# Komputerowe-Projektowanie-Lekow/pmarlo

Measured on AMD Instinct MI355X. Metric: frames/sec featurize->TICA->k-means->T-matrix, 1Mx64 synth; ITS rel-err, higher is better.
Workload: dtype f64; 1 GPU; synthetic 1000000 frames x 64 f32 features per GPU (AR(1) latents), TICA->10, k=500 (10 Lloyd iterations), lag=10, row-normalised T; frames_per_gpu=1000000, features=64, tica_dim=10, k=500, lag=10, kmeans_iters=10, parallelism=shards1

## Files before the change

### pmarlo_amd/csrc/kmeans.hip

```cpp
#include "common.h"
#include "wave.h"

#include <algorithm>
#include <cstdlib>

namespace {

constexpr int kThreads = 256;

template <typename T>
__device__ __forceinline__ double load_as_f64(const T* p) { return (double)(*p); }

struct FitState {
    double scale;
    double inv_scale;
    double absmax;
    double shift2;
    double tol2;
    double done;
    double n_iter;
    double inertia;
};

__device__ __forceinline__ long long to_fixed(double v, double scale) { return __double2ll_rn(v * scale); }
// ... 673 lines not shown

template <typename T, int KS, bool ACCUM>
msm_status launch_mfma(msm_ctx* ctx, const T* x, int64_t n, int d, int64_t ld, const double* centers, int k,
                       const double* mean, const double* stdv, int32_t* labels, double* mindist, const FitState* st,
                       unsigned long long* sums, unsigned long long* counts) {
    constexpr int NF = KS <= 16 ? 2 : 1;
    constexpr int kMT = KS <= 4 ? kMTNarrow : kMTWide;
    constexpr int TS = KS * 64 + 1;
    const size_t acc_bytes = ACCUM ? (size_t)k * (d + 1) * sizeof(unsigned long long) : 0;
    const int lds_acc = ACCUM && acc_bytes <= 64 * 1024;
    const size_t tile_budget = 150 * 1024 - (lds_acc ? acc_bytes : 0);
    int tile_k = (int)(tile_budget / ((TS + 16) * sizeof(double))) * 16;
    const int k16 = (k + 15) & ~15;
    if (tile_k > k16) tile_k = k16;
    if (tile_k < 16) tile_k = 16;
    if (tile_k < k16 && tile_k >= 32) tile_k &= ~31;
    const size_t lds = (size_t)(tile_k / 16) * (TS + 16) * sizeof(double) + (lds_acc ? acc_bytes : 0);
    const int64_t n_units = (n + 16 * NF - 1) / (16 * NF);
    const int waves = kMT / 64;
    const int grid = (int)std::min<int64_t>((n_units + waves - 1) / waves, (int64_t)ctx->n_cu);
    const bool multi = k > tile_k;
    const bool foldm = (d & 3) != 0;
    auto kern = multi ? (foldm ? kmeans_mfma_kernel<T, KS, NF, kMT, ACCUM, true, true>
                               : kmeans_mfma_kernel<T, KS, NF, kMT, ACCUM, false, true>)
                      : (foldm ? kmeans_mfma_kernel<T, KS, NF, kMT, ACCUM, true, false>
                               : kmeans_mfma_kernel<T, KS, NF, kMT, ACCUM, false, false>);
    double* chalf_g = nullptr;
    double* tile_img = nullptr;
    if (multi) {
        const size_t n_tiles_all = (size_t)k16 / 16;
        const size_t img_doubles = (n_tiles_all * TS + 1) & ~(size_t)1;
        msm_status rs = msm_reserve_aux(ctx, (img_doubles + k16) * sizeof(double));
        if (rs != MSM_OK) return rs;
        tile_img = (double*)ctx->aux;
        chalf_g = tile_img + img_doubles;
        if (foldm)
            hipLaunchKernelGGL((pack_tiles_kernel<KS, true>), dim3((unsigned)n_tiles_all), dim3(64), 0, ctx->stream, centers,
                               k, d, tile_img, chalf_g);
        else
            hipLaunchKernelGGL((pack_tiles_kernel<KS, false>), dim3((unsigned)n_tiles_all), dim3(64), 0, ctx->stream, centers,
                               k, d, tile_img, chalf_g);
    } else if (KS > 8) {
        msm_status rs = msm_reserve_aux(ctx, (size_t)k * sizeof(double));
        if (rs != MSM_OK) return rs;
        chalf_g = (double*)ctx->aux;
        hipLaunchKernelGGL(chalf_kernel, dim3((k + 255) / 256), dim3(256), 0, ctx->stream, centers, k, d, chalf_g);
    }
    if (getenv("MSM_KMEANS_DEBUG"))
        fprintf(stderr, "msm_kmeans: fp64 T=%s n=%lld d=%d k=%d KS=%d NF=%d MT=%d ACCUM=%d FOLD=%d MULTI=%d tile_k=%d lds_acc=%d grid=%d lds=%zu\n",
                sizeof(T) == 4 ? "f32" : "f64", (long long)n, d, k, KS, NF, kMT, (int)ACCUM, (int)foldm, (int)multi, tile_k,
                lds_acc, grid, lds);
    if (lds > 48 * 1024)
        MSM_HIP(ctx, hipFuncSetAttribute((const void*)kern, hipFuncAttributeMaxDynamicSharedMemorySize, (int)lds));
    hipLaunchKernelGGL(kern, dim3(grid), dim3(kMT), lds, ctx->stream, x, n, d, ld, centers, k, mean, stdv, tile_k,
                       labels, mindist, st, sums, counts, lds_acc, (const double*)chalf_g, (const double*)tile_img);
    MSM_CHECK_LAUNCH(ctx);
    return MSM_OK;
}

__global__ void mfma_bf16_probe_kernel(const uint16_t* __restrict__ A, const uint16_t* __restrict__ B,
                                       const float* __restrict__ C, float* __restrict__ D) {
    const int l = threadIdx.x, i = l & 15, q = l >> 4;
    A += (size_t)blockIdx.x * 512;
    B += (size_t)blockIdx.x * 512;
    C += (size_t)blockIdx.x * 256;
    D += (size_t)blockIdx.x * 256;
    v8bf a, b;
    for (int j = 0; j < 8; ++j) {
        a[j] = __builtin_bit_cast(__bf16, A[i * 32 + 8 * q + j]);
        b[j] = __builtin_bit_cast(__bf16, B[(8 * q + j) * 16 + i]);
    }
    v4f32 c;
    for (int r = 0; r < 4; ++r) c[r] = C[(4 * q + r) * 16 + i];
    c = __builtin_amdgcn_mfma_f32_16x16x32_bf16(a, b, c, 0, 0, 0);
    for (int r = 0; r < 4; ++r) D[(4 * q + r) * 16 + i] = c[r];
}

__global__ void mfma_f16_probe_kernel(const uint16_t* __restrict__ A, const uint16_t* __restrict__ B,
                                      const float* __restrict__ C, float* __restrict__ D) {
    const int l = threadIdx.x, i = l & 15, q = l >> 4;
    A += (size_t)blockIdx.x * 512;
    B += (size_t)blockIdx.x * 512;
    C += (size_t)blockIdx.x * 256;
    D += (size_t)blockIdx.x * 256;
    v8h a, b;
    for (int j = 0; j < 8; ++j) {
        a[j] = __builtin_bit_cast(_Float16, A[i * 32 + 8 * q + j]);
        b[j] = __builtin_bit_cast(_Float16, B[(8 * q + j) * 16 + i]);
    }
    v4f32 c;
    for (int r = 0; r < 4; ++r) c[r] = C[(4 * q + r) * 16 + i];
    c = __builtin_amdgcn_mfma_f32_16x16x32_f16(a, b, c, 0, 0, 0);
    for (int r = 0; r < 4; ++r) D[(4 * q + r) * 16 + i] = c[r];
}

bool filter_enabled() {
    static const bool on = [] {
        const char* e = getenv("MSM_KMEANS_FILTER");
        return !(e && e[0] == '0');
    }();
    return on;
}

size_t filter_image_bytes(int64_t n, int) { return (size_t)((n + 63) & ~(int64_t)63) * 16 * kFilterRowQ + 16; }

template <typename T>
msm_status launch_pack(msm_ctx* ctx, const T* x, int64_t n, int d, int64_t ld, const double* mean, const double* stdv,
                       const double* absmax, uint4* image) {
    const unsigned grid = (unsigned)((n + 255) / 256);
    if (!absmax) {
        uint4* tail = image + (size_t)((n + 63) & ~(int64_t)63) * kFilterRowQ;
        MSM_HIP(ctx, hipMemsetAsync(tail, 0, 8, ctx->stream));
        const int g = (int)std::min<int64_t>((n * d + 256 * 8 - 1) / (256 * 8), (int64_t)ctx->n_cu * 8);
        hipLaunchKernelGGL(filter_absmax_kernel<T>, dim3(g), dim3(256), 0, ctx->stream, x, n, d, ld, mean, stdv,
                           (unsigned long long*)tail);
        MSM_CHECK_LAUNCH(ctx);
        absmax = (const double*)tail;
    }
    const int dense = ld == d && ((uintptr_t)x & 15) == 0;
#define MSM_PACK_CASE(D)                                                                                              \
    case D:                                                                                                           \
        hipLaunchKernelGGL((kmeans_pack_kernel<T, D>), dim3(grid), dim3(256), 0, ctx->stream, x, n, ld, mean, stdv, absmax, \
                           image, dense);                                                                             \
        break
    switch (d) {
        MSM_PACK_CASE(1); MSM_PACK_CASE(2); MSM_PACK_CASE(3); MSM_PACK_CASE(4); MSM_PACK_CASE(5);
        MSM_PACK_CASE(6); MSM_PACK_CASE(7); MSM_PACK_CASE(8); MSM_PACK_CASE(9); MSM_PACK_CASE(10);
        default: return msm_fail(ctx, MSM_ERR_UNSUPPORTED, "k-means frame images need d <= %d (got %d)", kFilterMaxD, d);
    }
#undef MSM_PACK_CASE
    MSM_CHECK_LAUNCH(ctx);
    return MSM_OK;
}

msm_status filter_stats_buffer(msm_ctx* ctx, unsigned long long** out) {
    static_assert(sizeof(unsigned long long) == 8, "");
    if (!ctx->km_stats) {
        if (ctx->capturing) { *out = nullptr; return MSM_OK; }
        MSM_HIP(ctx, hipMalloc(&ctx->km_stats, 16));
        MSM_HIP(ctx, hipMemsetAsync(ctx->km_stats, 0, 16, ctx->stream));
    }
    *out = (unsigned long long*)ctx->km_stats;
    return MSM_OK;
}

template <typename T, int DP, bool ACCUM>
msm_status launch_filter_dp(msm_ctx* ctx, const T* x, int64_t n, int d, int64_t ld, const double* centers, int k,
                            const double* mean, const double* stdv, const uint4* image, int32_t* labels, double* mindist,
                            const FitState* st, unsigned long long* sums, unsigned long long* counts, double* upd_centers) {
    constexpr int NF = 4;
    const size_t lds = filter_lds_bytes(k, d, ACCUM);
    msm_status rs;
    const int64_t n_units = (n + 16 * NF - 1) / (16 * NF);
    const int kWaves = filter_waves(DP, ACCUM);
    const int grid = (int)std::min<int64_t>((n_units + kWaves - 1) / kWaves, (int64_t)ctx->n_cu);
    unsigned long long* stats = nullptr;
    rs = filter_stats_buffer(ctx, &stats);
    if (rs != MSM_OK) return rs;
    auto kern = mean ? kmeans_filter_kernel<T, DP, NF, ACCUM, true> : kmeans_filter_kernel<T, DP, NF, ACCUM, false>;
    if (lds > 48 * 1024)
        MSM_HIP(ctx, hipFuncSetAttribute((const void*)kern, hipFuncAttributeMaxDynamicSharedMemorySize, (int)lds));
    hipLaunchKernelGGL(kern, dim3(grid), dim3(64 * kWaves), lds, ctx->stream, x, n, d, ld, k, mean, stdv, image, centers,
                       labels, mindist, st, sums, counts, stats, stats ? upd_centers : nullptr,
                       stats ? (unsigned int*)(stats + 1) : nullptr);
    MSM_CHECK_LAUNCH(ctx);
    return MSM_OK;
}

template <typename T, bool ACCUM>
msm_status launch_filter(msm_ctx* ctx, const T* x, int64_t n, int d, int64_t ld, const double* centers, int k,
                         const double* mean, const double* stdv, const uint4* image, int32_t* labels, double* mindist,
                         const FitState* st, unsigned long long* sums, unsigned long long* counts, double* upd_centers) {
    if (filter_dp(d) == 4)
        return launch_filter_dp<T, 4, ACCUM>(ctx, x, n, d, ld, centers, k, mean, stdv, image, labels, mindist, st, sums,
                                             counts, upd_centers);
    return launch_filter_dp<T, 10, ACCUM>(ctx, x, n, d, ld, centers, k, mean, stdv, image, labels, mindist, st, sums, counts,
                                          upd_centers);
}

bool filter_fits(int k, int d, bool accum) { return filter_enabled() && d <= kFilterMaxD && filter_lds_bytes(k, d, accum) != 0; }

template <typename T, bool ACCUM>
msm_status dispatch_mfma(msm_ctx* ctx, const T* x, int64_t n, int d, int64_t ld, const double* centers, int k,
                         const double* mean, const double* stdv, int32_t* labels, double* mindist, const FitState* st,
                         unsigned long long* sums, unsigned long long* counts, const void* image = nullptr,
                         double* upd_centers = nullptr, bool* folded = nullptr) {
    if (folded) *folded = false;
    if (filter_fits(k, d, ACCUM)) {
        if (getenv("MSM_KMEANS_DEBUG"))
            fprintf(stderr, "msm_kmeans: filter T=%s n=%lld d=%d k=%d ACCUM=%d\n", sizeof(T) == 4 ? "f32" : "f64", (long long)n,
                    d, k, (int)ACCUM);
        if (!image) {
            msm_status rs = msm_reserve_km_image(ctx, filter_image_bytes(n, d));
            if (rs != MSM_OK) return rs;
            rs = launch_pack<T>(ctx, x, n, d, ld, mean, stdv, nullptr, (uint4*)ctx->km_image);
            if (rs != MSM_OK) return rs;
            image = ctx->km_image;
        }
        if (upd_centers && !(ACCUM && (int64_t)k * d <= kUpdateWide && (ctx->km_stats || !ctx->capturing))) upd_centers = nullptr;
        if (folded) *folded = upd_centers != nullptr;
        return launch_filter<T, ACCUM>(ctx, x, n, d, ld, centers, k, mean, stdv, (const uint4*)image, labels, mindist, st,
                                       sums, counts, upd_centers);
    }
#define MSM_MFMA_CASE(KSV) \
    if (d <= 4 * KSV)      \
        return launch_mfma<T, KSV, ACCUM>(ctx, x, n, d, ld, centers, k, mean, stdv, labels, mindist, st, sums, counts)
    MSM_MFMA_CASE(1);
    MSM_MFMA_CASE(2);
    MSM_MFMA_CASE(3);
    MSM_MFMA_CASE(4);
    MSM_MFMA_CASE(6);
    MSM_MFMA_CASE(8);
    MSM_MFMA_CASE(12);
    MSM_MFMA_CASE(16);
    MSM_MFMA_CASE(24);
    MSM_MFMA_CASE(32);
    MSM_MFMA_CASE(48);
    MSM_MFMA_CASE(64);
#undef MSM_MFMA_CASE
    return msm_fail(ctx, MSM_ERR_UNSUPPORTED, "k-means: d=%d > 256 not supported", d);
}

msm_status mfma_probe(msm_ctx* ctx, bool f16, const uint16_t* h_a, const uint16_t* h_b, const float* h_c, float* h_d,
                      int n_tiles) {
    if (!ctx) return MSM_ERR_INVALID;
    MSM_REQUIRE(ctx, n_tiles >= 1 && h_a && h_b && h_c && h_d, "msm_mfma_probe: bad arguments");
    const size_t na = (size_t)n_tiles * 512 * sizeof(uint16_t), nc = (size_t)n_tiles * 256 * sizeof(float);
    msm_status rs = msm_reserve_scratch(ctx, 2 * na + 2 * nc);
    if (rs != MSM_OK) return rs;
    unsigned char* base = (unsigned char*)ctx->scratch;
    uint16_t* d_a = (uint16_t*)base;
    uint16_t* d_b = (uint16_t*)(base + na);
    float* d_c = (float*)(base + 2 * na);
    float* d_d = (float*)(base + 2 * na + nc);
    MSM_HIP(ctx, hipMemcpyAsync(d_a, h_a, na, hipMemcpyHostToDevice, ctx->stream));
    MSM_HIP(ctx, hipMemcpyAsync(d_b, h_b, na, hipMemcpyHostToDevice, ctx->stream));
    MSM_HIP(ctx, hipMemcpyAsync(d_c, h_c, nc, hipMemcpyHostToDevice, ctx->stream));
    if (f16)
        hipLaunchKernelGGL(mfma_f16_probe_kernel, dim3((unsigned)n_tiles), dim3(64), 0, ctx->stream, d_a, d_b, d_c, d_d);
    else
        hipLaunchKernelGGL(mfma_bf16_probe_kernel, dim3((unsigned)n_tiles), dim3(64), 0, ctx->stream, d_a, d_b, d_c, d_d);
    MSM_CHECK_LAUNCH(ctx);
    MSM_HIP(ctx, hipMemcpyAsync(h_d, d_d, nc, hipMemcpyDeviceToHost, ctx->stream));
    MSM_HIP(ctx, hipStreamSynchronize(ctx->stream));
    return MSM_OK;
}

}

extern "C" {

static msm_status kmeans_assign_impl(msm_ctx* ctx, const void* d_x, msm_dtype dtype, int64_t n, int d, int64_t ld,
                                     const double* d_centers, int k, const double* d_mean, const double* d_std,
                                     const void* d_image, int32_t* d_labels, double* d_mindist) {
    if (!ctx) return MSM_ERR_INVALID;
    MSM_REQUIRE(ctx, n >= 0 && d >= 1 && k >= 1, "msm_kmeans_assign: need n >= 0, d >= 1, k >= 1");
    MSM_REQUIRE(ctx, ld >= d, "msm_kmeans_assign: ld (%lld) < d (%d)", (long long)ld, d);
    MSM_REQUIRE(ctx, (d_mean == nullptr) == (d_std == nullptr),
                "msm_kmeans_assign: mean and std must both be given or both be NULL");
    MSM_REQUIRE(ctx, dtype == MSM_F32 || dtype == MSM_F64, "msm_kmeans_assign: bad dtype");
    if (n == 0) return MSM_OK;
    MSM_REQUIRE(ctx, d_x && d_centers && d_labels, "msm_kmeans_assign: NULL pointer");
    if (dtype == MSM_F32)
        return dispatch_mfma<float, false>(ctx, (const float*)d_x, n, d, ld, d_centers, k, d_mean, d_std, d_labels,
                                           d_mindist, nullptr, nullptr, nullptr, d_image);
    return dispatch_mfma<double, false>(ctx, (const double*)d_x, n, d, ld, d_centers, k, d_mean, d_std, d_labels,
                                        d_mindist, nullptr, nullptr, nullptr, d_image);
}

msm_status msm_kmeans_assign(msm_ctx* ctx, const void* d_x, msm_dtype dtype, int64_t n, int d, int64_t ld,
                             const double* d_centers, int k, const double* d_mean, const double* d_std,
                             int32_t* d_labels, double* d_mindist) {
    return kmeans_assign_impl(ctx, d_x, dtype, n, d, ld, d_centers, k, d_mean, d_std, nullptr, d_labels, d_mindist);
}

msm_status msm_kmeans_assign_packed(msm_ctx* ctx, const void* d_x, msm_dtype dtype, int64_t n, int d, int64_t ld,
                                    const double* d_centers, int k, const double* d_mean, const double* d_std,
                                    const void* d_image, int32_t* d_labels, double* d_mindist) {
    return kmeans_assign_impl(ctx, d_x, dtype, n, d, ld, d_centers, k, d_mean, d_std, d_image, d_labels, d_mindist);
}

msm_status msm_kmeans_image_bytes(int64_t n, int d, size_t* out_bytes) {
    if (!out_bytes || n < 0 || d < 1) return MSM_ERR_INVALID;
    *out_bytes = d <= kFilterMaxD ? filter_image_bytes(n, d) : 0;
    return MSM_OK;
}

msm_status msm_kmeans_pack(msm_ctx* ctx, const void* d_x, msm_dtype dtype, int64_t n, int d, int64_t ld,
                           const double* d_mean, const double* d_std, void* d_image) {
    return msm_kmeans_pack_bounded(ctx, d_x, dtype, n, d, ld, d_mean, d_std, nullptr, d_image);
}

msm_status msm_kmeans_pack_bounded(msm_ctx* ctx, const void* d_x, msm_dtype dtype, int64_t n, int d, int64_t ld,
                                   const double* d_mean, const double* d_std, const double* d_absmax, void* d_image) {
    if (!ctx) return MSM_ERR_INVALID;
    MSM_REQUIRE(ctx, n >= 0 && d >= 1 && d <= kFilterMaxD && ld >= d, "msm_kmeans_pack: need 1 <= d <= %d, ld >= d",
                kFilterMaxD);
    MSM_REQUIRE(ctx, (d_mean == nullptr) == (d_std == nullptr), "msm_kmeans_pack: mean/std must come together");
    MSM_REQUIRE(ctx, dtype == MSM_F32 || dtype == MSM_F64, "msm_kmeans_pack: bad dtype");
    if (n == 0) return MSM_OK;
    MSM_REQUIRE(ctx, d_x && d_image, "msm_kmeans_pack: NULL pointer");
    MSM_REQUIRE(ctx, ((uintptr_t)d_image & 15) == 0, "msm_kmeans_pack: the image must be 16-byte aligned");
    if (dtype == MSM_F32)
        return launch_pack<float>(ctx, (const float*)d_x, n, d, ld, d_mean, d_std, d_absmax, (uint4*)d_image);
    return launch_pack<double>(ctx, (const double*)d_x, n, d, ld, d_mean, d_std, d_absmax, (uint4*)d_image);
}

// ... 191 lines not shown
```

### pmarlo_amd/csrc/kmeans_filter.h

```cpp
#pragma once

typedef __bf16 v8bf __attribute__((ext_vector_type(8)));
typedef _Float16 v8h __attribute__((ext_vector_type(8)));
typedef float v4f32 __attribute__((ext_vector_type(4)));

#ifdef MSM_KMF_WAVES
__host__ __device__ constexpr int filter_waves(int, bool) { return MSM_KMF_WAVES; }
#else
__host__ __device__ constexpr int filter_waves(int dp, bool heavy) { return dp == 10 && heavy ? 12 : 16; }
#endif
constexpr int kFilterMaxD = 10;
constexpr int kFilterRowQ = 3;
constexpr double kFilterHi = 1e18;
constexpr double kFilterScaledHi = 16384.0;
constexpr double kF16MinNormal = 6.103515625e-05;
constexpr int kFilterScaleTop = 13;
constexpr double kFilterKappa = 52.0 * 5.9604644775390625e-08;
constexpr float kPickEps = 20.0f * 5.9604644775390625e-08f;
constexpr float kPickFloor = 1e-30f;
constexpr float kUp20 = 1.0f + 9.5367431640625e-07f;
constexpr double kUp20d = 1.0 + 9.5367431640625e-07;

__host__ __device__ inline int filter_scale_exp(double amax) {
    if (!(amax > 0.0) || !(amax <= 1.7976931348623157e308)) return 0;
    const int q = ilogb(amax) + 1;
    const int e = kFilterScaleTop - q;
    return e < -60 ? -60 : (e > 60 ? 60 : e);
}

__device__ __forceinline__ double f16_round(double v) {
    const int q = ilogb(v) + 1;
    return ldexp(rint(ldexp(v, 11 - q)), q - 11);
}
__device__ __forceinline__ double f16_ceil(double v) {
    const int q = ilogb(v) + 1;
    return ldexp(ceil(ldexp(v, 11 - q)), q - 11);
}
__device__ __forceinline__ unsigned short f16_bits(double v) {
    return __builtin_bit_cast(unsigned short, (_Float16)(float)v);
}
__device__ __forceinline__ void f16_split2(double v, unsigned short& hi, unsigned short& lo, double& tiny) {
    hi = lo = 0;
    if (!(fabs(v) >= kF16MinNormal)) {
        tiny += fabs(v);
        return;
    }
    const double h = f16_round(v);
    const double r = v - h;
    hi = f16_bits(h);
    if (!(fabs(r) >= kF16MinNormal)) {
        tiny += fabs(r);
        return;
    }
    lo = f16_bits(f16_round(r));
}
__device__ __forceinline__ float f32_up(double v) {
    float f = (float)v;
    if ((double)f < v) f = __uint_as_float(__float_as_uint(f) + (f >= 0.0f ? 1u : ~0u));
    return f;
}

__host__ __device__ constexpr int filter_slot(int t, int f) { return f < 8 ? 8 * t + f : 24 + 2 * t + (f - 8); }
constexpr int kFilterSlotNorm = 31;
__device__ __forceinline__ int filter_piece(int q) { return q == 3 ? 2 : (q & 1); }

__device__ __forceinline__ float max3_f32(float a, float b, float c) { return __builtin_fmaxf(__builtin_fmaxf(a, b), c); }
__device__ __forceinline__ float med3_f32(float a, float b, float c) { return __builtin_amdgcn_fmed3f(a, b, c); }

template <typename T, int D>
__global__ __launch_bounds__(256) void kmeans_pack_kernel(const T* __restrict__ x, int64_t n, int64_t ld,
                                                         const double* __restrict__ mean,
                                                         const double* __restrict__ stdv, const double* absmax,
                                                         uint4* __restrict__ image, int dense) {
    constexpr int RQ = kFilterRowQ;
    constexpr int kOutStride = RQ;
    constexpr int kInBytes = 256 * D * (int)sizeof(T);
    constexpr int kOutBytes = 256 * kOutStride * 16;
    __shared__ __attribute__((aligned(16))) unsigned char stage[kOutBytes > kInBytes ? kOutBytes : kInBytes];
    const int64_t t0 = (int64_t)blockIdx.x * 256;
    const int64_t t = t0 + threadIdx.x;
    const int rows = (int)(n - t0 < 256 ? n - t0 : 256);
    const int64_t n_pad = (n + 63) & ~(int64_t)63;
    const int rows_out = (int)(n_pad - t0 < 256 ? n_pad - t0 : 256);
    const int ex = filter_scale_exp(*absmax);
    if (blockIdx.x == 0 && threadIdx.x == 0) reinterpret_cast<int*>(image + n_pad * RQ)[2] = ex;
    double v[D];
    if (dense) {
        const unsigned char* src = reinterpret_cast<const unsigned char*>(x + t0 * D);
        const int nbytes = rows * D * (int)sizeof(T);
        for (int b = threadIdx.x * 16; b + 16 <= nbytes; b += 256 * 16)
            *reinterpret_cast<uint4*>(stage + b) = *reinterpret_cast<const uint4*>(src + b);
        if (threadIdx.x < (nbytes & 15) / (int)sizeof(T)) {
            const int e = (nbytes & ~15) / (int)sizeof(T) + threadIdx.x;
            reinterpret_cast<T*>(stage)[e] = reinterpret_cast<const T*>(src)[e];
        }
        __syncthreads();
        const T* row = reinterpret_cast<const T*>(stage) + threadIdx.x * D;
#pragma unroll
        for (int f = 0; f < D; ++f) v[f] = threadIdx.x < rows ? (double)row[f] : 0.0;
        __syncthreads();
    } else {
        const T* row = x + (t < n ? t : n - 1) * ld;
#pragma unroll
        for (int f = 0; f < D; ++f) v[f] = load_as_f64(row + f);
    }
    bool ok = t < n;
#pragma unroll
    for (int f = 0; f < D; ++f) {
        if (mean) v[f] = (v[f] - mean[f]) / stdv[f];
        ok = ok && fabs(v[f]) <= kFilterHi;
        v[f] = ldexp(v[f], ex);
        ok = ok && fabs(v[f]) <= kFilterScaledHi;
    }
    unsigned short hi[D], lo[D];
    double q = 0.0, tiny = 0.0;
#pragma unroll
    for (int f = 0; f < D; ++f) {
        hi[f] = lo[f] = 0;
        if (ok) {
            q = fma(v[f], v[f], q);
            f16_split2(v[f], hi[f], lo[f], tiny);
        }
    }
    const unsigned short xn =
        ok ? f16_bits(f16_ceil(fmax((sqrt(q) + 2.0 * tiny / kFilterKappa) * kUp20d, kF16MinNormal))) : 0x7C00;
    unsigned short s[8 * RQ];
#pragma unroll
    for (int i = 0; i < 8 * RQ; ++i) s[i] = 0;
#pragma unroll
    for (int f = 0; f < D; ++f) {
        if (f < 8) {
            s[f] = hi[f];
            s[8 + f] = lo[f];
        } else {
            s[16 + f - 8] = s[20 + f - 8] = hi[f];
            s[18 + f - 8] = lo[f];
        }
    }
    s[23] = xn;
    uint4* mine = reinterpret_cast<uint4*>(stage) + threadIdx.x * kOutStride;
#pragma unroll
    for (int c = 0; c < RQ; ++c)
        mine[c] = make_uint4(s[8 * c + 0] | ((unsigned)s[8 * c + 1] << 16), s[8 * c + 2] | ((unsigned)s[8 * c + 3] << 16),
                             s[8 * c + 4] | ((unsigned)s[8 * c + 5] << 16), s[8 * c + 6] | ((unsigned)s[8 * c + 7] << 16));
    __syncthreads();
    uint4* dst = image + t0 * RQ;
    for (int c = threadIdx.x; c < rows_out * RQ; c += 256)
        dst[c] = reinterpret_cast<const uint4*>(stage)[(c / RQ) * kOutStride + (c % RQ)];
}

template <int DP>
struct FilterShape {
    static constexpr int RF = DP == 4 ? 8 : 12;
    static constexpr int kTileBytes = 1024 + 16 * RF * 4 + 16 * 4 + 16 * 8;
};
__host__ __device__ constexpr int filter_dp(int d) { return d <= 4 ? 4 : 10; }

constexpr int kStageRegs = (16 * kFilterMaxD + 63) / 64;
__device__ __forceinline__ int stage_row(int i, int d) { return (int)(((float)i + 0.5f) * (1.0f / (float)d)); }
template <int DP>
__device__ __forceinline__ void filter_stage_fetch(int tile, int lane, const double* __restrict__ centers, int k, int d,
                                                   double (&c)[kStageRegs], double (&rc)[DP]) {
#pragma unroll
    for (int u = 0; u < kStageRegs; ++u) {
        const int i = lane + 64 * u;
        const int r = stage_row(i, d), j = tile * 16 + r;
        c[u] = (i < 16 * d && j < k) ? centers[(size_t)tile * 16 * d + i] : 0.0;
    }
    const int jr = tile * 16 + lane;
#pragma unroll
    for (int f = 0; f < DP; ++f) rc[f] = (lane < 16 && jr < k && f < d) ? centers[(size_t)jr * d + f] : 0.0;
}
template <int DP>
__device__ __forceinline__ void filter_stage_build(int tile, int lane, unsigned short* simg, const double (&c)[kStageRegs],
                                                   const double (&rc)[DP], int k, int d, int ec, int exc,
                                                   float* __restrict__ tab, float* __restrict__ cz, double* __restrict__ hs,
                                                   int* __restrict__ any_bad) {
    using S = FilterShape<DP>;
    for (int i = lane; i < 64 * 4; i += 64) reinterpret_cast<unsigned*>(simg)[i] = 0u;
    for (int i = lane; i < 16 * S::RF; i += 64) tab[(size_t)tile * 16 * S::RF + i] = 0.0f;
    __builtin_amdgcn_fence(__ATOMIC_ACQ_REL, "wavefront");
    auto slot_addr = [&](int i, int sl) { return ((sl >> 3) * 16 + i) * 8 + (sl & 7); };
#pragma unroll
    for (int u = 0; u < kStageRegs; ++u) {
        const int i = lane + 64 * u;
        const int r = stage_row(i, d), f = i - r * d, j = tile * 16 + r;
        if (i < 16 * d && j < k) {
            tab[(size_t)j * S::RF + f] = (float)c[u];
            const double w = ldexp(c[u], ec);
            if (fabs(w) <= kFilterScaledHi) {
                unsigned short ch, cl;
                double tiny = 0.0;
                f16_split2(w, ch, cl, tiny);
                simg[slot_addr(r, filter_slot(0, f))] = ch;
                simg[slot_addr(r, filter_slot(1, f))] = ch;
                simg[slot_addr(r, filter_slot(2, f))] = cl;
            }
        }
    }
    __builtin_amdgcn_fence(__ATOMIC_ACQ_REL, "wavefront");
    int bad_row = 0;
    if (lane < 16) {
        const int j = tile * 16 + lane;
        float* row = tab + (size_t)j * S::RF;
        double h = __builtin_inf();
        if (j < k) {
            double a = 0.0, aw = 0.0, tiny = 0.0;
            bool ok = true;
#pragma unroll
            for (int f = 0; f < DP; ++f) {
                const double cf = rc[f];
                a = fma(cf, cf, a);
                const double w = ldexp(cf, ec);
                ok = ok && fabs(cf) <= kFilterHi && fabs(w) <= kFilterScaledHi;
                if (ok) {
                    aw = fma(w, w, aw);
                    const double r = fabs(w) >= kF16MinNormal ? fabs(w - f16_round(w)) : fabs(w);
                    if (!(r >= kF16MinNormal) || !(fabs(w) >= kF16MinNormal)) tiny += r;
                }
            }
            h = 0.5 * a;
            const double cval = ldexp(-(h - kFilterKappa * h), exc);
            ok = ok && fabs(cval) <= 0x1p100;
            if (!ok) bad_row = 1;
            cz[j] = ok ? f32_up(cval) : 0.0f;
            if (ok)
                simg[slot_addr(lane, kFilterSlotNorm)] =
                    f16_bits(f16_ceil(fmax((kFilterKappa * sqrt(aw) + 2.0 * tiny) * kUp20d, kF16MinNormal)));
            row[DP] = (float)h;
            row[DP + 1] = (float)(sqrt(a) * kUp20d);
        } else {
            cz[j] = -3.0e38f;
            row[DP] = 3.0e38f;
            row[DP + 1] = -3.0e38f;
        }
        hs[j] = h;
    }
    const bool bad = __any(bad_row != 0);
    if (bad && lane == 0) atomicOr(any_bad, 1);
}


template <typename T>
__global__ __launch_bounds__(256) void filter_absmax_kernel(const T* __restrict__ x, int64_t n, int d, int64_t ld,
                                                           const double* __restrict__ mean, const double* __restrict__ stdv,
                                                           unsigned long long* __restrict__ out_bits) {
    double m = 0.0;
    for (int64_t i = (int64_t)blockIdx.x * 256 + threadIdx.x; i < n * d; i += (int64_t)gridDim.x * 256) {
        const int64_t r = i / d;
        const int f = (int)(i - r * d);
        double v = load_as_f64(x + r * ld + f);
        if (mean) v = (v - mean[f]) / stdv[f];
        if (fabs(v) <= kFilterHi) m = fmax(m, fabs(v));
    }
    m = wave_max_f64(m);
    __shared__ double wm[4];
    if ((threadIdx.x & 63) == 0) wm[threadIdx.x >> 6] = m;
    __syncthreads();
    if (threadIdx.x == 0) {
        m = fmax(fmax(wm[0], wm[1]), fmax(wm[2], wm[3]));
        if (m > 0.0) atomicMax(out_bits, (unsigned long long)__double_as_longlong(m));
    }
}

template <typename T, int DP, bool WHITEN>
__device__ __forceinline__ void filter_load_frame(const T* __restrict__ x, int64_t ld, int d, bool vec_rows,
                                                  const double* __restrict__ mean, const double* __restrict__ stdv,
                                                  int64_t t, double (&z)[DP]) {
    const T* row = x + t * ld;
    if (vec_rows) {
        const double2* r2 = reinterpret_cast<const double2*>(row);
#pragma unroll
        for (int f2 = 0; f2 < DP / 2; ++f2) {
            const double2 v = r2[f2];
            z[2 * f2] = v.x;
            z[2 * f2 + 1] = v.y;
        }
    } else {
#pragma unroll
        for (int f = 0; f < DP; ++f) {
            const double v = load_as_f64(row + (f < d ? f : d - 1));
            z[f] = f < d ? v : 0.0;
        }
    }
    if constexpr (WHITEN) {
#pragma unroll
        for (int f = 0; f < DP; ++f) {
            const int fc = f < d ? f : d - 1;
            const double w = (z[f] - mean[fc]) / stdv[fc];
            z[f] = f < d ? w : 0.0;
        }
    }
}

template <int MT>
__device__ __forceinline__ void filter_close_iteration(const unsigned long long* sums, const unsigned long long* counts, int k,
                                                       int d, double* centers, FitState* st) {
    __shared__ double red[16];
    const int tid = threadIdx.x;
    const double inv_scale = st->inv_scale;
    for (int v0 = 0; v0 < 1024; v0 += MT) {
        const int v = v0 + tid;
        if (v < 1024) {
            double acc = 0.0;
            constexpr int CH = 4;
            for (int i0 = v; i0 < k * d; i0 += 1024 * CH) {
                long long cnt[CH], sm[CH];
                double old[CH];
#pragma unroll
                for (int c = 0; c < CH; ++c) {
                    const int i = i0 + c * 1024;
                    cnt[c] = 0;
                    if (i < k * d) {
                        cnt[c] = (long long)__hip_atomic_load(&counts[i / d], __ATOMIC_RELAXED, __HIP_MEMORY_SCOPE_AGENT);
                        sm[c] = (long long)__hip_atomic_load(&sums[i], __ATOMIC_RELAXED, __HIP_MEMORY_SCOPE_AGENT);
                        old[c] = centers[i];
                    }
                }
#pragma unroll
                for (int c = 0; c < CH; ++c)
                    if (cnt[c] > 0) {
                        const double c_new = (double)sm[c] * inv_scale / (double)cnt[c];
                        const double dlt = c_new - old[c];
                        acc = fma(dlt, dlt, acc);
                        centers[i0 + c * 1024] = c_new;
                    }
            }
            for (int off = 32; off > 0; off >>= 1) acc += __shfl_down(acc, off, 64);
            if ((v & 63) == 0) red[v >> 6] = acc;
        }
    }
    __syncthreads();
    if (tid == 0) {
        double t = 0.0;
        for (int i = 0; i < 16; ++i) t += red[i];
        st->shift2 = t;
        st->n_iter += 1.0;
        if (t <= st->tol2) st->done = 1.0;
    }
}

template <typename T, int DP, int NF, bool ACCUM, bool WHITEN>
__global__ __launch_bounds__(64 * filter_waves(DP, ACCUM)) void kmeans_filter_kernel(
    const T* __restrict__ x, int64_t n, int d, int64_t ld, int k, const double* __restrict__ mean,
    const double* __restrict__ stdv, const uint4* __restrict__ image, const double* __restrict__ centers,
    int32_t* __restrict__ labels,
    double* __restrict__ mindist, const FitState* __restrict__ st, unsigned long long* __restrict__ sums,
    unsigned long long* __restrict__ counts, unsigned long long* __restrict__ n_scanned, double* upd_centers,
    unsigned int* __restrict__ ticket) {
    using S = FilterShape<DP>;
    constexpr int kFilterWaves = filter_waves(DP, ACCUM);
    constexpr int kMT = 64 * kFilterWaves, RF = S::RF, RQ = kFilterRowQ;
    static_assert(NF == 4, "one frame group per lane quarter: a unit is 64 frames, one per lane in the candidate pick");
    extern __shared__ __attribute__((aligned(16))) unsigned char smem_raw[];
    if constexpr (ACCUM) {
        if (st->done != 0.0) return;
    }
    const int k16 = (k + 15) & ~15;
    const int n_tiles = ((k16 / 16) + 1) & ~1;
    uint4* img = reinterpret_cast<uint4*>(smem_raw);
    float* tab = reinterpret_cast<float*>(img + (size_t)n_tiles * 64);
    float* cz = tab + (size_t)n_tiles * 16 * RF;
    double* hs = reinterpret_cast<double*>(cz + (size_t)n_tiles * 16);
    unsigned long long* lsum = reinterpret_cast<unsigned long long*>(hs + (size_t)n_tiles * 16);
    unsigned long long* lcnt = lsum + (ACCUM ? (size_t)k * d : 0);
    __shared__ int unit_ctr;
    __shared__ int any_bad;
    __shared__ unsigned long long cmax_bits;
    const int tid = threadIdx.x, lane = tid & 63, wave = __builtin_amdgcn_readfirstlane(tid >> 6);
    const int j16 = lane & 15, q = lane >> 4;
    const double scale = ACCUM ? st->scale : 0.0;
    if (tid == 0) {
        unit_ctr = kFilterWaves;
        any_bad = 0;
        cmax_bits = 0ull;
    }
    KSTAMP_INIT
    if constexpr (ACCUM) {
        for (int i = tid; i < k * (d + 1); i += kMT) lsum[i] = 0ull;
    }
    __syncthreads();
    constexpr int kUnit = 16 * NF;
    const int64_t n_units = (n + kUnit - 1) / kUnit;
    const int64_t units_per_block = (n_units + gridDim.x - 1) / gridDim.x;
    const int64_t u_begin = (int64_t)blockIdx.x * units_per_block;
    const int64_t u_end = min(n_units, u_begin + units_per_block);
    const int voff = j16 * RQ + filter_piece(q);
    const int ex = reinterpret_cast<const int*>(image + (size_t)((n + 63) & ~(int64_t)63) * RQ)[2];

    int64_t unit = u_begin + wave;
    v8h b[NF];
    auto load_images = [&](int64_t un) {
        const uint4* ub = image + un * (kUnit * RQ);
#pragma unroll
        for (int u = 0; u < NF; ++u) b[u] = __builtin_bit_cast(v8h, ub[voff + u * 16 * RQ]);
    };
    if (unit < u_end) load_images(unit);

    {
        double cm = 0.0;
        for (int i = tid; i < k * d; i += kMT) cm = fmax(cm, fabs(centers[i]));
        cm = wave_max_f64(cm);
        if (lane == 0 && cm > 0.0) atomicMax(&cmax_bits, (unsigned long long)__double_as_longlong(cm));
    }
    __syncthreads();
    const int ec = __builtin_amdgcn_readfirstlane(filter_scale_exp(__longlong_as_double((long long)cmax_bits)));
    const int exc = ex + ec;
    for (int t = wave; t < n_tiles; t += 2 * kFilterWaves) {
        const int t2 = t + kFilterWaves;
        double c0[kStageRegs], c1[kStageRegs], r0[DP], r1[DP];
        filter_stage_fetch<DP>(t, lane, centers, k, d, c0, r0);
        if (t2 < n_tiles) filter_stage_fetch<DP>(t2, lane, centers, k, d, c1, r1);
        filter_stage_build<DP>(t, lane, reinterpret_cast<unsigned short*>(img + (size_t)t * 64), c0, r0, k, d, ec, exc, tab, cz,
                               hs, &any_bad);
        if (t2 < n_tiles)
            filter_stage_build<DP>(t2, lane, reinterpret_cast<unsigned short*>(img + (size_t)t2 * 64), c1, r1, k, d, ec, exc, tab,
                                   cz, hs, &any_bad);
    }
    __syncthreads();
    const float inv_scale_u = __int_as_float((127 - exc) << 23);
    const bool all_scan = __builtin_amdgcn_readfirstlane(any_bad) != 0;
    KSTAMP(0);

    unsigned long long my_scans = 0;
    const bool vec_rows = sizeof(T) == 8 && d == DP && ((ld * sizeof(T)) & 15) == 0 && (((uintptr_t)x) & 15) == 0;
    const int iters = n_tiles / 2;
    constexpr int kNone = 0x7fffffff;

    auto load_frame = [&](int64_t t, double (&z)[DP]) { filter_load_frame<T, DP, WHITEN>(x, ld, d, vec_rows, mean, stdv, t, z); };
    auto score64 = [&](const double* crow, int c, const double (&z)[DP]) {
        double a = 0.0;
#pragma unroll
        for (int f = 0; f < DP; ++f)
            if (f < d) a = fma(crow[f], z[f], a);
        return a - hs[c];
    };
    auto write_label = [&](int64_t t, int bidx, double bm, const double (&z)[DP]) {
        labels[t] = bidx;
        if (mindist) {
            double zsq = 0.0;
#pragma unroll
            for (int f = 0; f < DP; ++f) zsq = fma(z[f], z[f], zsq);
            const double md = -2.0 * bm + zsq;
            mindist[t] = md > 0.0 ? md : 0.0;
        }
    };
    auto commit_scan = [&](int64_t t, int sbi, double sbest, const double (&zz)[DP], int old_s) {
        if constexpr (ACCUM) {
            if (!labels || old_s != sbi) {
#pragma unroll
                for (int f = 0; f < DP; ++f) {
                    if (f < d && lane == f) {
                        const unsigned long long fx = (unsigned long long)to_fixed(zz[f], scale);
                        atomicAdd(&lsum[(size_t)sbi * d + f], fx);
                        if (old_s >= 0) atomicAdd(&lsum[(size_t)old_s * d + f], 0ull - fx);
                    }
                }
                if (lane == 0) {
                    atomicAdd(&lcnt[sbi], 1ull);
                    if (old_s >= 0) atomicAdd(&lcnt[old_s], ~0ull);
                    if (labels) labels[t] = sbi;
                }
            }
        } else {
            if (lane == 0) write_label(t, sbi, sbest, zz);
        }
    };
    auto scan_frame = [&](int64_t t) {
        double zz[DP];
        load_frame(t, zz);
        double sbest = -__builtin_inf();
        int sbi = kNone;
        for (int c = lane; c < k; c += 64) {
            const double sc = score64(centers + (size_t)c * d, c, zz);
            if (sc > sbest) { sbest = sc; sbi = c; }
        }
#pragma unroll
        for (int off = 1; off < 64; off <<= 1) {
            const double ob = __shfl_xor(sbest, off, 64);
            const int oi = __shfl_xor(sbi, off, 64);
            if (ob > sbest || (ob == sbest && oi < sbi)) { sbest = ob; sbi = oi; }
        }
        if (sbi >= k) { sbi = 0; sbest = -__builtin_inf(); }
        int old_s = -1;
        if constexpr (ACCUM) {
            if (labels) old_s = labels[t];
        }
        commit_scan(t, sbi, sbest, zz, old_s);
#ifdef MSM_KMF_DIAG_COUNT
        if (MSM_KMF_DIAG_COUNT == 1) ++my_scans;
#else
        ++my_scans;
#endif
    };

    while (unit < u_end) {
        int nt = 0;
        if (lane == 0) nt = atomicAdd(&unit_ctr, 1);
        const int64_t nxt = u_begin + __builtin_amdgcn_readfirstlane(nt);
        KSTAMP_VM(1);
        float b1[NF], b2[NF];
        int bp[NF];
#pragma unroll
        for (int u = 0; u < NF; ++u) { b1[u] = -__builtin_inff(); b2[u] = -__builtin_inff(); bp[u] = 0; }
#ifdef MSM_KMF_DIAG_NOTILE
        for (int it = 0; it < (iters < 9 ? iters : 9); ++it) {
#else
        for (int it = 0; it < iters; ++it) {
#endif
            const int jt = 2 * it;
            const v8h aa = __builtin_bit_cast(v8h, img[(jt + 0) * 64 + lane]);
            const v8h ab = __builtin_bit_cast(v8h, img[(jt + 1) * 64 + lane]);
            const v4f32 ca = *reinterpret_cast<const v4f32*>(cz + (jt + 0) * 16 + 4 * q);
            const v4f32 cb = *reinterpret_cast<const v4f32*>(cz + (jt + 1) * 16 + 4 * q);
            v4f32 acca[NF], accb[NF];
#pragma unroll
            for (int u = 0; u < NF; ++u) {
                acca[u] = __builtin_amdgcn_mfma_f32_16x16x32_f16(aa, b[u], ca, 0, 0, 0);
                accb[u] = __builtin_amdgcn_mfma_f32_16x16x32_f16(ab, b[u], cb, 0, 0, 0);
            }
#pragma unroll
            for (int u = 0; u < NF; ++u) {
                float m = max3_f32(b2[u], acca[u][0], acca[u][1]);
                m = max3_f32(m, acca[u][2], acca[u][3]);
                m = max3_f32(m, accb[u][0], accb[u][1]);
                m = max3_f32(m, accb[u][2], accb[u][3]);
                const bool better = m > b1[u];
                b2[u] = med3_f32(b1[u], b2[u], m);
                b1[u] = hw_max_f32(b1[u], m);
                bp[u] = better ? jt : bp[u];
            }
        }
        KSTAMP(2);
        bool guard[NF];
#pragma unroll
        for (int u = 0; u < NF; ++u) guard[u] = q == 3 && __builtin_bit_cast(unsigned short, b[u][7]) == 0x7C00;
        if (nxt < u_end) load_images(nxt);
        const int64_t f0 = unit * kUnit + lane;
        const bool fok = f0 < n;
        const int64_t fr = fok ? f0 : n - 1;
        int old = -1;
        if constexpr (ACCUM) {
            if (labels) old = labels[fr];
        }
        double z[DP];
        load_frame(fr, z);
        int cd = kNone;
        float Ru = __builtin_inff();
#ifdef MSM_KMF_DIAG_NOCROSS
        cd = bp[0] | (q << 16);
        Ru = b2[0] + b1[1] + b1[2] + b1[3] + b2[1] + b2[2] + b2[3] + (guard[0] | guard[1] | guard[2] | guard[3] ? 1.f : 0.f) + (float)(bp[1] + bp[2] + bp[3]);
#else
#pragma unroll
        for (int u = 0; u < NF; ++u) {
            const float M1 = xrow_max_f32(b1[u]);
            const int code_u = xrow_min_i32(b1[u] == M1 ? ((q << 16) | bp[u]) : kNone);
            const int gs = code_u >> 16;
            float r = q == gs ? b2[u] : b1[u];
            if (guard[u]) r = __builtin_inff();
            const float R_u = xrow_max_f32(r);
            cd = q == u ? code_u : cd;
            Ru = q == u ? R_u : Ru;
        }
#endif
        Ru = __builtin_fmaf(Ru, inv_scale_u, 1.40129846e-45f);
        KSTAMP(3);
        const int gs = cd >> 16, pstar = cd & 0xffff;
        const int base = min(pstar * 16 + 4 * gs, n_tiles * 16 - 20);
        float pz[DP];
        float qz = 0.f;
#pragma unroll
        for (int f = 0; f < DP; ++f) {
            pz[f] = (float)z[f];
            qz = __builtin_fmaf(pz[f], pz[f], qz);
        }
        const bool z_bad = !(qz < __builtin_inff());
        const float zn = hw_max_f32(__builtin_amdgcn_sqrtf(qz) * kUp20, 1.0f);
        float s1 = -__builtin_inff(), s2 = -__builtin_inff(), sbmax = 0.f;
        int i1 = 0;
#ifndef MSM_KMF_DIAG_NOPICK
        const float* p_row = tab + (size_t)base * RF;
#pragma unroll
        for (int c = 0; c < 8; ++c) {
            const float4* r4 = reinterpret_cast<const float4*>(p_row + ((c & 3) + 16 * (c >> 2)) * RF);
            float a = 0.f, h, cn;
            if constexpr (DP == 4) {
                const float4 r0 = r4[0], r1 = r4[1];
                a = __builtin_fmaf(r0.x, pz[0], a);
                a = __builtin_fmaf(r0.y, pz[1], a);
                a = __builtin_fmaf(r0.z, pz[2], a);
                a = __builtin_fmaf(r0.w, pz[3], a);
                h = r1.x;
                cn = r1.y;
            } else {
                const float4 r0 = r4[0], r1 = r4[1], r2 = r4[2];
                a = __builtin_fmaf(r0.x, pz[0], a);
                a = __builtin_fmaf(r0.y, pz[1], a);
                a = __builtin_fmaf(r0.z, pz[2], a);
                a = __builtin_fmaf(r0.w, pz[3], a);
                a = __builtin_fmaf(r1.x, pz[4], a);
                a = __builtin_fmaf(r1.y, pz[5], a);
                a = __builtin_fmaf(r1.z, pz[6], a);
                a = __builtin_fmaf(r1.w, pz[7], a);
                a = __builtin_fmaf(r2.x, pz[8], a);
                a = __builtin_fmaf(r2.y, pz[9], a);
                h = r2.z;
                cn = r2.w;
            }
            const float s = a - h;
            sbmax = hw_max_f32(sbmax, __builtin_fmaf(zn, cn, h));
            const bool better = s > s1;
            s2 = med3_f32(s1, s2, s);
            s1 = hw_max_f32(s1, s);
            i1 = better ? c : i1;
        }
#endif
        const float e = __builtin_fmaf(kPickEps, sbmax, kPickFloor);
        const int jw = base + (i1 & 3) + 16 * (i1 >> 2);
        const bool certified = !all_scan && !z_bad && cd != kNone && jw < k && s1 - s2 > 2.0f * e && s1 - e > Ru;
        const int lab = jw;
#if defined(MSM_KMF_DIAG_NOSCAN) || defined(MSM_KMF_DIAG_NOQUEUE)
        unsigned long long todo = 0;
#else
        unsigned long long todo = __ballot(fok && !certified);
#endif
        KSTAMP(4);
#ifdef MSM_KMF_DIAG_NOCOMMIT
        if (fok && certified && cd == 12345) {
#else
        if (fok && certified) {
#endif
            if constexpr (ACCUM) {
                if (!labels || old != lab) {
#pragma unroll
                    for (int f = 0; f < DP; ++f) {
                        if (f < d) {
                            const unsigned long long fx = (unsigned long long)to_fixed(z[f], scale);
                            atomicAdd(&lsum[(size_t)lab * d + f], fx);
                            if (old >= 0) atomicAdd(&lsum[(size_t)old * d + f], 0ull - fx);
                        }
                    }
                    atomicAdd(&lcnt[lab], 1ull);
                    if (old >= 0) atomicAdd(&lcnt[old], ~0ull);
                    if (labels) labels[f0] = lab;
                }
            } else {
                if (mindist) write_label(f0, lab, score64(centers + (size_t)lab * d, lab, z), z);
                else labels[f0] = lab;
            }
        }
        KSTAMP(5);
        while (todo) {
            const int jf = __builtin_ctzll(todo);
            todo &= todo - 1;
            const int64_t t = ((int64_t)__builtin_amdgcn_readlane((int)(f0 >> 32), jf) << 32) |
                              (unsigned)__builtin_amdgcn_readlane((int)f0, jf);
            const bool plain = all_scan || __builtin_amdgcn_readlane((int)(z_bad || !(Ru < __builtin_inff())), jf) != 0;
            if (plain) {
                scan_frame(t);
                continue;
            }
            float zf[DP];
#pragma unroll
            for (int f = 0; f < DP; ++f) zf[f] = __int_as_float(__builtin_amdgcn_readlane(__float_as_int(pz[f]), jf));
            const float znj = __int_as_float(__builtin_amdgcn_readlane(__float_as_int(zn), jf));
            float t1 = -__builtin_inff(), t2 = -__builtin_inff(), t3 = -__builtin_inff(), sbl = 0.f;
            int c1 = 0, c2 = 0;
            for (int c = lane; c < n_tiles * 16; c += 64) {
                const float4* r4 = reinterpret_cast<const float4*>(tab + (size_t)c * RF);
                float a = 0.f, h, cn;
                if constexpr (DP == 4) {
                    const float4 r0 = r4[0], r1 = r4[1];
                    a = __builtin_fmaf(r0.x, zf[0], a);
                    a = __builtin_fmaf(r0.y, zf[1], a);
                    a = __builtin_fmaf(r0.z, zf[2], a);
                    a = __builtin_fmaf(r0.w, zf[3], a);
                    h = r1.x;
                    cn = r1.y;
                } else {
                    const float4 r0 = r4[0], r1 = r4[1], r2 = r4[2];
                    a = __builtin_fmaf(r0.x, zf[0], a);
                    a = __builtin_fmaf(r0.y, zf[1], a);
                    a = __builtin_fmaf(r0.z, zf[2], a);
                    a = __builtin_fmaf(r0.w, zf[3], a);
                    a = __builtin_fmaf(r1.x, zf[4], a);
                    a = __builtin_fmaf(r1.y, zf[5], a);
                    a = __builtin_fmaf(r1.z, zf[6], a);
                    a = __builtin_fmaf(r1.w, zf[7], a);
                    a = __builtin_fmaf(r2.x, zf[8], a);
                    a = __builtin_fmaf(r2.y, zf[9], a);
                    h = r2.z;
                    cn = r2.w;
                }
                const float sc = a - h;
                sbl = hw_max_f32(sbl, __builtin_fmaf(znj, cn, h));
                if (sc > t1) { t3 = t2; t2 = t1; c2 = c1; t1 = sc; c1 = c; }
                else if (sc > t2) { t3 = t2; t2 = sc; c2 = c; }
                else t3 = hw_max_f32(t3, sc);
            }
            double rowa[DP], rowb[DP];
            {
                const double* ca = centers + (size_t)(c1 < k ? c1 : 0) * d;
                const double* cb = centers + (size_t)(c2 < k ? c2 : 0) * d;
#pragma unroll
                for (int f = 0; f < DP; ++f) {
                    rowa[f] = f < d ? ca[f] : 0.0;
                    rowb[f] = f < d ? cb[f] : 0.0;
                }
            }
            const float top = wave_max_f32(t1), sbw = wave_max_f32(sbl);
            const float band = top - 2.0f * __builtin_fmaf(kPickEps, sbw, kPickFloor);
            const unsigned long long in1 = __ballot(t1 >= band);
            if (__any(t3 >= band) || in1 == 0ull) {
                scan_frame(t);
                continue;
            }
            double zz[DP];
#pragma unroll
            for (int f = 0; f < DP; ++f) {
                const long long bits = __double_as_longlong(z[f]);
                zz[f] = __longlong_as_double((long long)(((unsigned long long)(unsigned)__builtin_amdgcn_readlane((int)(bits >> 32), jf) << 32) |
                                                         (unsigned)__builtin_amdgcn_readlane((int)bits, jf)));
            }
            const int old_t = __builtin_amdgcn_readlane(old, jf);
            int sbi;
            double sbest = 0.0;
            const bool two = __any(t2 >= band) || __builtin_popcountll(in1) > 1;
            if (!two && !(mindist && !ACCUM)) {
                sbi = __builtin_amdgcn_readlane(c1, __builtin_ctzll(in1));
            } else {
                double m1 = -__builtin_inf();
                int i1b = kNone;
                auto chain = [&](const double (&row)[DP], int c) {
                    double a = 0.0;
#pragma unroll
                    for (int f = 0; f < DP; ++f) a = fma(row[f], zz[f], a);
                    return a - hs[c];
                };
                if (t1 >= band && c1 < k) { m1 = chain(rowa, c1); i1b = c1; }
                if (t2 >= band && c2 < k) {
                    const double m2 = chain(rowb, c2);
                    if (m2 > m1 || (m2 == m1 && c2 < i1b)) { m1 = m2; i1b = c2; }
                }
                sbest = wave_max_f64(m1);
                sbi = wave_min_i32(m1 == sbest ? i1b : kNone);
                if (sbi >= k) {
                    scan_frame(t);
                    continue;
                }
            }
            commit_scan(t, sbi, sbest, zz, old_t);
#ifdef MSM_KMF_DIAG_COUNT
            if (MSM_KMF_DIAG_COUNT == 2 && two) ++my_scans;
#else
            ++my_scans;
#endif
        }
        KSTAMP(6);
        unit = nxt;
    }
    KSTAMP(7);
    if (n_scanned && lane == 0 && my_scans) atomicAdd(n_scanned, my_scans);
    if constexpr (ACCUM) {
        __syncthreads();
        for (int i = tid; i < k * d; i += kMT)
            if (lsum[i]) atomicAdd(&sums[i], lsum[i]);
        for (int i = tid; i < k; i += kMT)
            if (lcnt[i]) atomicAdd(&counts[i], lcnt[i]);
        if (upd_centers) {
            __shared__ int is_last;
            asm volatile("s_waitcnt vmcnt(0)" ::: "memory");
            __syncthreads();
            if (tid == 0) {
                const unsigned t = __hip_atomic_fetch_add(ticket, 1u, __ATOMIC_RELAXED, __HIP_MEMORY_SCOPE_AGENT);
                is_last = t == gridDim.x - 1;
                if (is_last) __hip_atomic_store(ticket, 0u, __ATOMIC_RELAXED, __HIP_MEMORY_SCOPE_AGENT);
            }
            __syncthreads();
            if (is_last) filter_close_iteration<kMT>(sums, counts, k, d, upd_centers, const_cast<FitState*>(st));
        }
    }
    KSTAMP_FLUSH
}

static inline size_t filter_lds_bytes(int k, int d, bool accum) {
    if (d > kFilterMaxD) return 0;
    const int k16 = (k + 15) & ~15;
    const int n_tiles = ((k16 / 16) + 1) & ~1;
    const size_t tile_bytes = filter_dp(d) == 4 ? FilterShape<4>::kTileBytes : FilterShape<10>::kTileBytes;
    const size_t total = (size_t)n_tiles * tile_bytes + (accum ? (size_t)k * (d + 1) * sizeof(unsigned long long) : 0);
    const size_t cap = 160 * 1024 - 64;
    return total <= cap ? total : 0;
}
```

Before: 702.1 million frames/s.

## Cut register pressure in accumulating k-means filter by deferring f64 frame loads

In the accumulating k-means filter, each frame is now loaded straight into f32 registers for the candidate pick. The f64 copy is re-read from memory only when a frame's label actually changes, or when a frame falls back to the exact scan. The prefetch of center rows for the second staged tile is moved after the first tile's build, so its live range is shorter. The wave count per block now also depends on row dtype and whitening, so f64 unwhitened rows get 16 waves instead of 12. The aim is fewer live VGPRs and higher occupancy, at the cost of redundant global reloads for reassigned or ambiguous frames.

```diff
diff --git a/pmarlo_amd/csrc/kmeans.hip b/pmarlo_amd/csrc/kmeans.hip
--- a/pmarlo_amd/csrc/kmeans.hip
+++ b/pmarlo_amd/csrc/kmeans.hip
@@ -849,7 +849,7 @@
     const size_t lds = filter_lds_bytes(k, d, ACCUM);
     msm_status rs;
     const int64_t n_units = (n + 16 * NF - 1) / (16 * NF);
-    const int kWaves = filter_waves(DP, ACCUM);
+    const int kWaves = filter_waves(DP, ACCUM, sizeof(T) == 8, mean != nullptr);
     const int grid = (int)std::min<int64_t>((n_units + kWaves - 1) / kWaves, (int64_t)ctx->n_cu);
     unsigned long long* stats = nullptr;
     rs = filter_stats_buffer(ctx, &stats);
diff --git a/pmarlo_amd/csrc/kmeans_filter.h b/pmarlo_amd/csrc/kmeans_filter.h
--- a/pmarlo_amd/csrc/kmeans_filter.h
+++ b/pmarlo_amd/csrc/kmeans_filter.h
@@ -5,9 +5,11 @@
 typedef float v4f32 __attribute__((ext_vector_type(4)));
 
 #ifdef MSM_KMF_WAVES
-__host__ __device__ constexpr int filter_waves(int, bool) { return MSM_KMF_WAVES; }
+__host__ __device__ constexpr int filter_waves(int, bool, bool, bool) { return MSM_KMF_WAVES; }
 #else
-__host__ __device__ constexpr int filter_waves(int dp, bool heavy) { return dp == 10 && heavy ? 12 : 16; }
+__host__ __device__ constexpr int filter_waves(int dp, bool accum, bool f64_rows, bool whiten) {
+    return dp == 10 && accum && (!f64_rows || whiten) ? 12 : 16;
+}
 #endif
 constexpr int kFilterMaxD = 10;
 constexpr int kFilterRowQ = 3;
@@ -158,18 +160,27 @@
 
 constexpr int kStageRegs = (16 * kFilterMaxD + 63) / 64;
 __device__ __forceinline__ int stage_row(int i, int d) { return (int)(((float)i + 0.5f) * (1.0f / (float)d)); }
-template <int DP>
-__device__ __forceinline__ void filter_stage_fetch(int tile, int lane, const double* __restrict__ centers, int k, int d,
-                                                   double (&c)[kStageRegs], double (&rc)[DP]) {
+__device__ __forceinline__ void filter_stage_fetch_tile(int tile, int lane, const double* __restrict__ centers, int k, int d,
+                                                        double (&c)[kStageRegs]) {
 #pragma unroll
     for (int u = 0; u < kStageRegs; ++u) {
         const int i = lane + 64 * u;
         const int r = stage_row(i, d), j = tile * 16 + r;
         c[u] = (i < 16 * d && j < k) ? centers[(size_t)tile * 16 * d + i] : 0.0;
     }
+}
+template <int DP>
+__device__ __forceinline__ void filter_stage_fetch_rows(int tile, int lane, const double* __restrict__ centers, int k, int d,
+                                                        double (&rc)[DP]) {
     const int jr = tile * 16 + lane;
 #pragma unroll
     for (int f = 0; f < DP; ++f) rc[f] = (lane < 16 && jr < k && f < d) ? centers[(size_t)jr * d + f] : 0.0;
+}
+template <int DP>
+__device__ __forceinline__ void filter_stage_fetch(int tile, int lane, const double* __restrict__ centers, int k, int d,
+                                                   double (&c)[kStageRegs], double (&rc)[DP]) {
+    filter_stage_fetch_tile(tile, lane, centers, k, d, c);
+    filter_stage_fetch_rows<DP>(tile, lane, centers, k, d, rc);
 }
 template <int DP>
 __device__ __forceinline__ void filter_stage_build(int tile, int lane, unsigned short* simg, const double (&c)[kStageRegs],
@@ -293,6 +304,32 @@
     }
 }
 
+template <typename T, int DP, bool WHITEN>
+__device__ __forceinline__ void filter_load_frame_f32(const T* __restrict__ x, int64_t ld, int d, bool vec_rows,
+                                                      const double* __restrict__ mean, const double* __restrict__ stdv,
+                                                      int64_t t, float (&pz)[DP]) {
+    const T* row = x + t * ld;
+    auto narrow = [&](double v, int f) {
+        if constexpr (WHITEN) {
+            const int fc = f < d ? f : d - 1;
+            v = (v - mean[fc]) / stdv[fc];
+        }
+        return f < d ? (float)v : 0.0f;
+    };
+    if (vec_rows) {
+        const double2* r2 = reinterpret_cast<const double2*>(row);
+#pragma unroll
+        for (int f2 = 0; f2 < DP / 2; ++f2) {
+            const double2 v = r2[f2];
+            pz[2 * f2] = narrow(v.x, 2 * f2);
+            pz[2 * f2 + 1] = narrow(v.y, 2 * f2 + 1);
+        }
+    } else {
+#pragma unroll
+        for (int f = 0; f < DP; ++f) pz[f] = narrow(load_as_f64(row + (f < d ? f : d - 1)), f);
+    }
+}
+
 template <int MT>
 __device__ __forceinline__ void filter_close_iteration(const unsigned long long* sums, const unsigned long long* counts, int k,
                                                        int d, double* centers, FitState* st) {
@@ -341,7 +378,7 @@
 }
 
 template <typename T, int DP, int NF, bool ACCUM, bool WHITEN>
-__global__ __launch_bounds__(64 * filter_waves(DP, ACCUM)) void kmeans_filter_kernel(
+__global__ __launch_bounds__(64 * filter_waves(DP, ACCUM, sizeof(T) == 8, WHITEN)) void kmeans_filter_kernel(
     const T* __restrict__ x, int64_t n, int d, int64_t ld, int k, const double* __restrict__ mean,
     const double* __restrict__ stdv, const uint4* __restrict__ image, const double* __restrict__ centers,
     int32_t* __restrict__ labels,
@@ -349,7 +386,7 @@
     unsigned long long* __restrict__ counts, unsigned long long* __restrict__ n_scanned, double* upd_centers,
     unsigned int* __restrict__ ticket) {
     using S = FilterShape<DP>;
-    constexpr int kFilterWaves = filter_waves(DP, ACCUM);
+    constexpr int kFilterWaves = filter_waves(DP, ACCUM, sizeof(T) == 8, WHITEN);
     constexpr int kMT = 64 * kFilterWaves, RF = S::RF, RQ = kFilterRowQ;
     static_assert(NF == 4, "one frame group per lane quarter: a unit is 64 frames, one per lane in the candidate pick");
     extern __shared__ __attribute__((aligned(16))) unsigned char smem_raw[];
@@ -410,9 +447,15 @@
         const int t2 = t + kFilterWaves;
         double c0[kStageRegs], c1[kStageRegs], r0[DP], r1[DP];
         filter_stage_fetch<DP>(t, lane, centers, k, d, c0, r0);
-        if (t2 < n_tiles) filter_stage_fetch<DP>(t2, lane, centers, k, d, c1, r1);
+        if (t2 < n_tiles) {
+            filter_stage_fetch_tile(t2, lane, centers, k, d, c1);
+            if constexpr (!ACCUM) filter_stage_fetch_rows<DP>(t2, lane, centers, k, d, r1);
+        }
         filter_stage_build<DP>(t, lane, reinterpret_cast<unsigned short*>(img + (size_t)t * 64), c0, r0, k, d, ec, exc, tab, cz,
                                hs, &any_bad);
+        if constexpr (ACCUM) {
+            if (t2 < n_tiles) filter_stage_fetch_rows<DP>(t2, lane, centers, k, d, r1);
+        }
         if (t2 < n_tiles)
             filter_stage_build<DP>(t2, lane, reinterpret_cast<unsigned short*>(img + (size_t)t2 * 64), c1, r1, k, d, ec, exc, tab,
                                    cz, hs, &any_bad);
@@ -428,6 +471,9 @@
     constexpr int kNone = 0x7fffffff;
 
     auto load_frame = [&](int64_t t, double (&z)[DP]) { filter_load_frame<T, DP, WHITEN>(x, ld, d, vec_rows, mean, stdv, t, z); };
+    auto load_frame_f32 = [&](int64_t t, float (&pz)[DP]) {
+        filter_load_frame_f32<T, DP, WHITEN>(x, ld, d, vec_rows, mean, stdv, t, pz);
+    };
     auto score64 = [&](const double* crow, int c, const double (&z)[DP]) {
         double a = 0.0;
 #pragma unroll
@@ -544,7 +590,9 @@
             if (labels) old = labels[fr];
         }
         double z[DP];
-        load_frame(fr, z);
+        float pz[DP];
+        if constexpr (ACCUM) load_frame_f32(fr, pz);
+        else load_frame(fr, z);
         int cd = kNone;
         float Ru = __builtin_inff();
 #ifdef MSM_KMF_DIAG_NOCROSS
@@ -567,11 +615,10 @@
         KSTAMP(3);
         const int gs = cd >> 16, pstar = cd & 0xffff;
         const int base = min(pstar * 16 + 4 * gs, n_tiles * 16 - 20);
-        float pz[DP];
         float qz = 0.f;
 #pragma unroll
         for (int f = 0; f < DP; ++f) {
-            pz[f] = (float)z[f];
+            if constexpr (!ACCUM) pz[f] = (float)z[f];
             qz = __builtin_fmaf(pz[f], pz[f], qz);
         }
         const bool z_bad = !(qz < __builtin_inff());
@@ -632,6 +679,7 @@
 #endif
             if constexpr (ACCUM) {
                 if (!labels || old != lab) {
+                    load_frame(f0, z);
 #pragma unroll
                     for (int f = 0; f < DP; ++f) {
                         if (f < d) {
@@ -716,11 +764,15 @@
                 continue;
             }
             double zz[DP];
-#pragma unroll
-            for (int f = 0; f < DP; ++f) {
-                const long long bits = __double_as_longlong(z[f]);
-                zz[f] = __longlong_as_double((long long)(((unsigned long long)(unsigned)__builtin_amdgcn_readlane((int)(bits >> 32), jf) << 32) |
-                                                         (unsigned)__builtin_amdgcn_readlane((int)bits, jf)));
+            if constexpr (ACCUM) {
+                load_frame(t, zz);
+            } else {
+#pragma unroll
+                for (int f = 0; f < DP; ++f) {
+                    const long long bits = __double_as_longlong(z[f]);
+                    zz[f] = __longlong_as_double((long long)(((unsigned long long)(unsigned)__builtin_amdgcn_readlane((int)(bits >> 32), jf) << 32) |
+                                                             (unsigned)__builtin_amdgcn_readlane((int)bits, jf)));
+                }
             }
             const int old_t = __builtin_amdgcn_readlane(old, jf);
             int sbi;
```

Result: no change. 708.1 million frames/s (median of 6 runs) (+0.9%).
